# actionml/universal-recommender

Hardware: NVIDIA H100
Metric: CCO train events/sec to indicator model (higher is better)
Workload: dtype int32+f64

## Files before the change

universal_recommender_b200/csrc/cco_api.cu:

```cuda
#include <cuda_runtime.h>
#include <dlfcn.h>
#include <stdarg.h>
#include <stdio.h>
#include <stdlib.h>
#include <string.h>

#include <algorithm>
#include <charconv>
#include <cmath>
#include <functional>
#include <cub/cub.cuh>
#include <nvtx3/nvToolsExt.h>
#include <condition_variable>
#include <mutex>
#include <string>
#include <thread>
#include <unordered_map>
#include <vector>

#include "../../include/cco_b200.h"
#include "cco_kernels.cuh"
#include "cco_sampler.cuh"
#include "cco_format.cuh"
#include "cco_strings.cuh"
#include "cco_json.cuh"
#include "cco_events.cuh"
#include "cco_queries.cuh"
#include "cco_results.cuh"
#include "cco_index_pages.cuh"
#include "cco_index_write.cuh"
#include "cco_refresh.cuh"
#include "cco_intern.cuh"

namespace cco {

static thread_local char g_err[512] = "";
static int set_error(int code, const char *fmt, ...) {
  va_list ap;
  va_start(ap, fmt);
  vsnprintf(g_err, sizeof g_err, fmt, ap);
  va_end(ap);
  return code;
}
#define CK(expr)                                                                                      \
  do {                                                                                                \
    cudaError_t _e = (expr);                                                                          \
    if (_e != cudaSuccess)                                                                            \
      return set_error(_e == cudaErrorMemoryAllocation ? CCO_E_OOM : CCO_E_CUDA, "%s: %s (%s:%d)", #expr, \
                       cudaGetErrorString(_e), __FILE__, __LINE__);                                   \
  } while (0)
#define CKR(expr)            \
  do {                       \
    int _r = (expr);         \
    if (_r != CCO_OK) return _r; \
  } while (0)

typedef struct ncclComm *ncclComm_t;
typedef struct { char internal[128]; } ncclUniqueId;
struct Nccl {
  void *h = nullptr;
  int (*GetUniqueId)(ncclUniqueId *) = nullptr;
  int (*CommInitRank)(ncclComm_t *, int, ncclUniqueId, int) = nullptr;
  int (*CommInitAll)(ncclComm_t *, int, const int *) = nullptr;
  int (*CommDestroy)(ncclComm_t) = nullptr;
  int (*AllReduce)(const void *, void *, size_t, int, int, ncclComm_t, cudaStream_t) = nullptr;
  int (*AllGather)(const void *, void *, size_t, int, ncclComm_t, cudaStream_t) = nullptr;
  int (*Broadcast)(const void *, void *, size_t, int, int, ncclComm_t, cudaStream_t) = nullptr;
  int (*GroupStart)() = nullptr;
  int (*GroupEnd)() = nullptr;
  const char *(*GetErrorString)(int) = nullptr;
};
static Nccl g_nccl;
static std::mutex g_nccl_mu;
static int load_nccl() {
  std::lock_guard<std::mutex> lk(g_nccl_mu);
  if (g_nccl.h) return CCO_OK;
  void *h = dlopen("libnccl.so.2", RTLD_NOW | RTLD_GLOBAL);
  if (!h) h = dlopen("libnccl.so", RTLD_NOW | RTLD_GLOBAL);
  if (!h) return set_error(CCO_E_NCCL, "cannot load libnccl.so.2: %s", dlerror());
#define SYM(field, name)                                                         \
  *(void **)(&g_nccl.field) = dlsym(h, name);                                    \
  if (!g_nccl.field) return set_error(CCO_E_NCCL, "libnccl: missing symbol %s", name);
  SYM(GetUniqueId, "ncclGetUniqueId")
  SYM(CommInitRank, "ncclCommInitRank")
  SYM(CommInitAll, "ncclCommInitAll")
  SYM(CommDestroy, "ncclCommDestroy")
  SYM(AllReduce, "ncclAllReduce")
  SYM(AllGather, "ncclAllGather")
  SYM(Broadcast, "ncclBroadcast")
  SYM(GroupStart, "ncclGroupStart")
  SYM(GroupEnd, "ncclGroupEnd")
  SYM(GetErrorString, "ncclGetErrorString")
#undef SYM
  g_nccl.h = h;
// ... 324 lines not shown
  c->launches++;
  ar.release(tmp);
  ar.release(kb.Alternate());
  ar.release(vb.Alternate());
  *k = kb.Current();
  *v = vb.Current();
  return CCO_OK;
}
static int bits_for(long long n) {
  int b = 1;
  while ((1LL << b) < n) ++b;
  return b;
}

static int keys_to_csr(cco_ctx *c, Arena &ar, unsigned long long *k0, unsigned long long *k1, long long n, int bits, long long n_valid,
                       long long n_rows, int32_t *col, long long *rp, long long *n_unique) {
  cudaStream_t s = c->stream;
  cub::DoubleBuffer<unsigned long long> db(k0, k1);
  size_t tb = 0;
  CK(cub::DeviceRadixSort::SortKeys(nullptr, tb, db, n, 0, bits, s));
  void *tmp;
  CKR(ar.alloc((char **)&tmp, tb));
  CK(cub::DeviceRadixSort::SortKeys(tmp, tb, db, n, 0, bits, s));
  ar.release(tmp);
  unsigned long long *sorted = db.Current(), *other = db.Alternate();
  uint32_t *flag, *pos;
  CKR(ar.alloc(&flag, n_valid + 1));
  CKR(ar.alloc(&pos, n_valid + 1));
  CK(cudaMemsetAsync(flag + n_valid, 0, 4, s));
  k_unique_flags<<<grid_for(n_valid, 256, c->sm_count), 256, 0, s>>>(n_valid, sorted, flag);
  CKR(exclusive_sum(c, ar, flag, pos, n_valid + 1));
  uint32_t nuq = 0;
  CKR(mail_fetch(c, &nuq, pos + n_valid, 4));
  k_unique_scatter<<<grid_for(n_valid, 256, c->sm_count), 256, 0, s>>>(n_valid, sorted, flag, pos, other, col);
  CKR(mail_wait(c));
  k_rowptr_from_keys<<<grid_for(n_rows + 1, 256, c->sm_count), 256, 0, s>>>(n_rows, nuq, other, rp);
  c->launches += 3;
  ar.release(flag);
  ar.release(pos);
  *n_unique = nuq;
  return CCO_OK;
}

static int canonicalize_device(cco_ctx *c, Arena &ar, DevRaw &m) {
  if (m.nnz == 0) return CCO_OK;
  unsigned long long *k0, *k1;
  CKR(ar.alloc(&k0, m.nnz));
  CKR(ar.alloc(&k1, m.nnz));
  k_expand_keys<<<grid_for(m.n_rows * kSG, 256, c->sm_count), 256, 0, c->stream>>>(m.n_rows, m.rp, m.col, k0);
  c->launches++;
  long long n_unique = 0;
  CKR(keys_to_csr(c, ar, k0, k1, m.nnz, 32 + bits_for(m.n_rows), m.nnz, m.n_rows, m.col + m.q_base, m.rp, &n_unique));
  m.col += m.q_base;
  m.q_base = 0;
  m.nnz = n_unique;
  CK(cudaGetLastError());
  ar.release(k0);
  ar.release(k1);
  return CCO_OK;
}

struct HeavyRows {
  int32_t *list = nullptr;
  int *n = nullptr;
};
static int list_heavy_rows(cco_ctx *c, Arena &ar, const DevRaw &raw, HeavyRows *h) {
  CKR(ar.alloc(&h->list, std::max<long long>(raw.n_rows, 1)));
  CKR(ar.alloc(&h->n, 1));
  CK(cudaMemsetAsync(h->n, 0, 4, c->stream));
  if (raw.n_rows > 0) {
    k_list_heavy_rows<<<grid_for(raw.n_rows, 256, c->sm_count), 256, 0, c->stream>>>(raw.n_rows, raw.rp, h->list, h->n);
    c->launches++;
  }
  return CCO_OK;
}
static void launch_check(cco_ctx *c, const DevRaw &raw, const HeavyRows &h, int *flags) {
  if (raw.n_rows <= 0) return;
  const long long q_lo = raw.q_base, q_hi = raw.q_base + raw.nnz;
  k_check_rows<kSG><<<grid_for(raw.n_rows * kSG, 256, c->sm_count), 256, 0, c->stream>>>(raw.n_rows, raw.n_cols, raw.rp, raw.col, q_lo, q_hi,
                                                                                       nullptr, nullptr, flags);
  k_check_rows<32><<<c->sm_count * 4, 256, 0, c->stream>>>(raw.n_rows, raw.n_cols, raw.rp, raw.col, q_lo, q_hi, h.list, h.n, flags);
  c->launches += 2;
}
struct SampleScratch {
  unsigned long long *col_thr = nullptr;
  uint8_t *keep = nullptr;
};
static int sample_scratch(cco_ctx *c, Arena &ar, const DevRaw &raw, const int32_t *raw_counts, int32_t m, SampleScratch *sc) {
  CKR(ar.alloc(&sc->col_thr, std::max<int32_t>(raw.n_cols, 1)));
  CKR(ar.alloc(&sc->keep, std::max<long long>(raw.nnz, 1)));
  if (raw.n_cols > 0) {
    k_col_thresholds<<<grid_for(raw.n_cols, 256, c->sm_count, 4), 256, 0, c->stream>>>(raw.n_cols, raw_counts, m, sc->col_thr);
    c->launches++;
  }
  return CCO_OK;
}
static void launch_count(cco_ctx *c, const DevRaw &raw, const SampleScratch &sc, int32_t m, int32_t seed, uint32_t flags, const int *bad,
                         uint32_t *kept, int32_t *new_counts) {
  if (raw.n_rows <= 0 || raw.nnz <= 0) return;
  const long long q_lo = raw.q_base, q_hi = raw.q_base + raw.nnz;
  const long long n_chunks = (raw.nnz + kSampleChunk - 1) / kSampleChunk;
  k_sample_count<<<grid_for(n_chunks * 32, 256, c->sm_count), 256, 0, c->stream>>>(raw.n_rows, raw.row_base, raw.rp, raw.col, raw.n_cols, q_lo, q_hi,
                                                                                  sc.col_thr, m, seed, flags, bad, kept, new_counts, sc.keep);
  c->launches++;
}
static int launch_write(cco_ctx *c, Arena &ar, const DevRaw &raw, const SampleScratch &sc, int32_t *dst) {
  if (raw.n_rows <= 0 || raw.nnz <= 0) return CCO_OK;
  long long *n_sel;
  CKR(ar.alloc(&n_sel, 1));
  size_t tb = 0;
  CK(cub::DeviceSelect::Flagged(nullptr, tb, raw.col + raw.q_base, sc.keep, dst, n_sel, (long long)raw.nnz, c->stream));
  void *tmp;
  CKR(ar.alloc((char **)&tmp, tb));
  CK(cub::DeviceSelect::Flagged(tmp, tb, raw.col + raw.q_base, sc.keep, dst, n_sel, (long long)raw.nnz, c->stream));
  ar.release(tmp);
  c->launches += 2;
  return CCO_OK;
}

constexpr int kHistCopies = 16;
static bool hist_fits_smem(const cco_ctx *c, int32_t n_cols) { return ((size_t)n_cols + 1) / 2 * 4 <= c->smem_optin; }
static int count_raw_columns(cco_ctx *c, Arena &ar, const std::vector<DevRaw> &raw, const std::vector<long long> &col_off, const cudaEvent_t *ready,
                             int *verdict, int32_t **counts_out) {
  cudaStream_t s = c->stream;
  const int n_mats = (int)raw.size();
  const long long total_cols = col_off[n_mats];
  const long long copy_stride = std::max<long long>(total_cols, 1);
  bool copies = false;
  for (int i = 0; i < n_mats; ++i) copies = copies || (raw[i].n_rows > 0 && !hist_fits_smem(c, raw[i].n_cols));
  const int n_copies = copies ? kHistCopies : 1;
  int32_t *counts;
  CKR(ar.alloc(&counts, (size_t)copy_stride * n_copies));
  CK(cudaMemsetAsync(counts, 0, sizeof(int32_t) * (size_t)copy_stride * n_copies, s));
  *counts_out = counts;
  std::vector<int> fit;
  for (int i = 0; i < n_mats; ++i)
    if (raw[i].n_rows > 0 && hist_fits_smem(c, raw[i].n_cols)) fit.push_back(i);
  for (size_t b0 = 0; b0 < fit.size(); b0 += kHistSegs) {
    const size_t b1 = std::min(fit.size(), b0 + kHistSegs);
    HistBatch hb{};
    long long nnz_sum = 0;
    int32_t max_cols = 0;
    for (size_t t = b0; t < b1; ++t) {
      nnz_sum += raw[fit[t]].nnz;
      max_cols = std::max(max_cols, raw[fit[t]].n_cols);
    }
    const size_t smem = ((size_t)max_cols + 1) / 2 * 4;
    const int per_sm = std::max(1, std::min<int>(2048 / kHistThreads, (int)(c->smem_optin / std::max<size_t>(smem + 1024, 1))));
    const long long target = (long long)c->sm_count * per_sm;
    for (size_t t = b0; t < b1; ++t) {
      const int i = fit[t];
      if (ready) CK(cudaStreamWaitEvent(s, ready[i], 0));
      const long long share = nnz_sum > 0 ? (target * raw[i].nnz + nnz_sum - 1) / nnz_sum : 1;
      const long long need = (raw[i].nnz + kHistMinEntries - 1) / kHistMinEntries;
      HistSeg &g = hb.seg[hb.n++];
      g.col = raw[i].col + raw[i].q_base;
      g.rp = raw[i].rp;
      g.nnz = raw[i].nnz;
      g.n_rows = raw[i].n_rows;
      g.q_lo = raw[i].q_base;
      g.q_hi = raw[i].q_base + raw[i].nnz;
      g.counts = counts + col_off[i];
      g.verdict = verdict ? verdict + 2 * i : nullptr;
      g.n_cols = raw[i].n_cols;
      g.cta0 = hb.cta_end;
      hb.cta_end += (int32_t)std::max(1LL, std::min(share, need));
    }
    CK(cudaFuncSetAttribute(k_col_counts_smem, cudaFuncAttributeMaxDynamicSharedMemorySize, (int)smem));
    k_col_counts_smem<<<hb.cta_end, kHistThreads, smem, s>>>(hb);
    c->launches++;
  }
  for (int i = 0; i < n_mats && copies; ++i) {
    if (raw[i].n_rows == 0 || hist_fits_smem(c, raw[i].n_cols)) continue;
    if (ready) CK(cudaStreamWaitEvent(s, ready[i], 0));
    int *v = verdict ? verdict + 2 * i : nullptr;
    if (v) {
      k_check_row_ptr<<<grid_for(raw[i].n_rows, 256, c->sm_count), 256, 0, s>>>(raw[i].n_rows, raw[i].rp, raw[i].q_base, raw[i].q_base + raw[i].nnz, v);
      c->launches++;
    }
    if (raw[i].nnz > 0) {
      k_col_histogram_flat<true><<<grid_for(raw[i].nnz, 256, c->sm_count), 256, 0, s>>>(raw[i].nnz, raw[i].col + raw[i].q_base, raw[i].n_cols,
                                                                                       counts + col_off[i], kHistCopies, copy_stride, v);
      c->launches++;
    }
  }
  if (copies) {
    k_sum_copies<<<grid_for(total_cols, 256, c->sm_count), 256, 0, s>>>(total_cols, kHistCopies, copy_stride, counts);
    c->launches++;
  }
  if (ready)
    for (int i = 0; i < n_mats; ++i) CK(cudaStreamWaitEvent(s, ready[i], 0));
  return CCO_OK;
}

static int nccl_check(int rc, const char *what) {
  if (rc != 0) return set_error(CCO_E_NCCL, "%s: %s", what, g_nccl.GetErrorString(rc));
  return CCO_OK;
}

static int downsample_all(cco_ctx *c, Arena &ar, const std::vector<DevRaw> &raw, const int *d_check , long long U,
                          const int32_t *raw_counts, int32_t *marg_all, const std::vector<long long> &col_off,
                          const cco_indicator_params_t *params, int32_t seed, uint32_t flags, std::vector<DevMat> &dm,
                          const cudaEvent_t *stage_ev ) {
  cudaStream_t s = c->stream;
  const int W = c->world, r = c->rank, n_mats = (int)raw.size();
  const long long S = (U + W - 1) / W;
  std::vector<uint32_t *> kept(n_mats, nullptr);
  std::vector<SampleScratch> sc(n_mats);
  for (int i = 0; i < n_mats; ++i) {
    DevMat *out = &dm[i];
    out->n_rows = U;
    out->n_cols = raw[i].n_cols;
    out->marg = marg_all + col_off[i];
    CKR(ar.alloc(&kept[i], (size_t)(W * S + 1)));
    CKR(ar.alloc(&out->rp, U + 1));
    CK(cudaMemsetAsync(kept[i], 0, sizeof(uint32_t) * (size_t)(W * S + 1), s));
    CKR(sample_scratch(c, ar, raw[i], raw_counts + col_off[i], params[i].max_interactions, &sc[i]));
    launch_count(c, raw[i], sc[i], params[i].max_interactions, seed, flags, d_check + 2 * i, kept[i], out->marg);
  }
  CK(cudaEventRecord(stage_ev[0], s));
  if (W > 1) {
    if (S > 0) {
      g_nccl.GroupStart();
      for (int i = 0; i < n_mats; ++i) {
        int rc = g_nccl.AllGather(kept[i] + (size_t)r * S, kept[i], (size_t)S, kNcclUint32, c->comm, s);
        if (rc != 0) { g_nccl.GroupEnd(); return nccl_check(rc, "ncclAllGather(kept counts)"); }
      }
      CKR(nccl_check(g_nccl.GroupEnd(), "ncclGroupEnd(kept counts)"));
    }
    if (col_off[n_mats] > 0)
      CKR(nccl_check(g_nccl.AllReduce(marg_all, marg_all, (size_t)col_off[n_mats], kNcclInt32, kNcclSum, c->comm, s), "ncclAllReduce(marginals)"));
  }
  std::vector<uint32_t> edge((size_t)n_mats * (W + 1), 0);
  for (int i = 0; i < n_mats; ++i) {
    CKR(exclusive_sum(c, ar, kept[i], dm[i].rp, U + 1));
    ar.release(kept[i]);
    if (W > 1)
      for (int q = 0; q <= W; ++q) CKR(mail_fetch(c, &edge[(size_t)i * (W + 1) + q], dm[i].rp + std::min<long long>((long long)q * S, U), 4));
  }
  CK(cudaEventRecord(stage_ev[1], s));
  if (W > 1) CKR(mail_wait(c));
  std::vector<long long> cap(n_mats, 0);
  std::vector<int32_t *> gathered(n_mats, nullptr);
  for (int i = 0; i < n_mats; ++i) {
    if (W == 1) {
      CKR(ar.alloc(&dm[i].col, std::max<long long>(raw[i].nnz, 1)));
      CKR(launch_write(c, ar, raw[i], sc[i], dm[i].col));
    } else {
      for (int q = 0; q < W; ++q) cap[i] = std::max<long long>(cap[i], (long long)edge[(size_t)i * (W + 1) + q + 1] - edge[(size_t)i * (W + 1) + q]);
      CKR(ar.alloc(&dm[i].col, std::max<long long>(edge[(size_t)i * (W + 1) + W], 1)));
      if (cap[i] > 0) {
        CKR(ar.alloc(&gathered[i], (size_t)(cap[i] * W)));
        CKR(launch_write(c, ar, raw[i], sc[i], gathered[i] + (size_t)r * cap[i]));
      }
    }
    ar.release(sc[i].col_thr);
    ar.release(sc[i].keep);
  }
  CK(cudaEventRecord(stage_ev[2], s));
  if (W > 1) {
    g_nccl.GroupStart();
    for (int i = 0; i < n_mats; ++i) {
      if (!gathered[i]) continue;
      int rc = g_nccl.AllGather(gathered[i] + (size_t)r * cap[i], gathered[i], (size_t)cap[i], kNcclInt32, c->comm, s);
      if (rc != 0) { g_nccl.GroupEnd(); return nccl_check(rc, "ncclAllGather(column blocks)"); }
    }
    CKR(nccl_check(g_nccl.GroupEnd(), "ncclGroupEnd(column blocks)"));
    for (int i = 0; i < n_mats; ++i) {
      if (!gathered[i]) continue;
      dim3 grid((unsigned)std::max(1, std::min(c->sm_count * 8 / W, 1024)), (unsigned)W);
      k_pack_blocks<<<grid, 256, 0, s>>>(W, S, U, cap[i], dm[i].rp, gathered[i], dm[i].col);
      c->launches++;
      ar.release(gathered[i]);
    }
  }
  CK(cudaEventRecord(stage_ev[3], s));
  CK(cudaGetLastError());
  return CCO_OK;
}


struct BinCfg {
  int group;
  int slots;
  int cap;
  int cbuf;
  int caux, keep_max, final_max;
  bool dense;
  bool bitmap;
  bool sorted;
  int bm_words;
  size_t region;
  size_t smem;
  int ctas_per_sm;
};

static int next_pow2(int x) {
  int p = 1;
  while (p < x) p <<= 1;
  return p;
}

template <int GROUP>
static int launch_rows_t(cco_ctx *c, const RowArgs &a, BinCfg &cfg, cudaStream_t st) {
  constexpr int CTA = GROUP == 32 ? 64 : GROUP;
  int occ = 1;
  void (*kern)(const RowArgs) = cfg.dense ? k_rows<GROUP, true> : k_rows<GROUP, false>;
  if constexpr (GROUP == 512 || GROUP == 256)
    if (cfg.bitmap) kern = k_rows<GROUP, false, true>;
  if constexpr (GROUP == 32)
    if (cfg.sorted) kern = k_rows<32, false, false, true>;
  CK(cudaFuncSetAttribute(kern, cudaFuncAttributeMaxDynamicSharedMemorySize, (int)cfg.smem));
  CK(cudaOccupancyMaxActiveBlocksPerMultiprocessor(&occ, kern, CTA, cfg.smem));
  kern<<<c->sm_count * std::max(occ, 1) * 4, CTA, cfg.smem, st>>>(a);
  cfg.ctas_per_sm = occ;
  c->launches++;
  CK(cudaGetLastError());
  return CCO_OK;
}
static int launch_rows(cco_ctx *c, const RowArgs &a, BinCfg &cfg, cudaStream_t st) {
  switch (cfg.group) {
    case 1024: return launch_rows_t<1024>(c, a, cfg, st);
    case 512: return launch_rows_t<512>(c, a, cfg, st);
    case 256: return launch_rows_t<256>(c, a, cfg, st);
    case 128: return launch_rows_t<128>(c, a, cfg, st);
    case 32: return launch_rows_t<32>(c, a, cfg, st);
  }
  return set_error(CCO_E_INVALID_ARG, "internal: bad bin config");
}

static BinCfg make_cfg(cco_ctx *c, int group, int want_slots, int top_k, int n_cols_b) {
  BinCfg f;
  const int groups = group == 32 ? 2 : 1;
  f.group = group;
  f.final_max = next_pow2(top_k);
  f.cbuf = next_pow2(top_k + std::max(group, 128) + (group == 32 ? 64 : 0));
  if (group == 32 && top_k + 32 <= 96) f.cbuf = 128;
  f.keep_max = std::max(f.final_max, (f.cbuf - group) / 2);
  f.caux = group == 32 ? 0 : f.keep_max;
  size_t fixed = (size_t)(f.cbuf + f.caux) * 16 + 2 * 256 + 512 + 1024 + (size_t)(group / 32) * 256;
  size_t avail = (c->smem_optin - 1024) / groups;
// ... 6038 lines not shown
    if (len[i] < 1 || len[i] > 32) return set_error(CCO_E_CUDA, "text %lld has length %d", (long long)i, len[i]);
    memcpy(bytes + offsets[i], slot.data() + 32 * (size_t)i, (size_t)len[i]);
    offsets[i + 1] = offsets[i] + len[i];
  }
  return CCO_OK;
}

int cco_debug_downsample(cco_ctx_t *c, const cco_csr_t *m, int32_t max_interactions, int32_t seed, uint32_t flags,
                         int64_t **row_ptr, int32_t **col_idx, int32_t *raw_col_counts, int32_t *new_col_counts) {
  if (!c || !m || !row_ptr || !col_idx) return set_error(CCO_E_INVALID_ARG, "null argument");
  if (c->world != 1 || !c->members.empty()) return set_error(CCO_E_UNSUPPORTED, "debug entries need a single-GPU context");
  cco_indicator_params_t prm = {max_interactions, 1, 0, 0.0};
  CKR(validate_host(1, m, &prm));
  CK(cudaSetDevice(c->device));
  mail_reset(c);
  c->ev_timing_used = c->ev_plain_used = 0;
  cco_dataset *ds = nullptr;
  CKR(dataset_upload(c, 1, m, flags, &ds));
  struct DG { cco_dataset *d; ~DG() { dataset_release(d); } } dg{ds};
  Arena ar(c->stream);
  Prepared p;
  CKR(prepare(c, ar, ds, &prm, seed, flags, &p));
  const DevMat &dm = p.dm[0];
  std::vector<uint32_t> rp32((size_t)m->n_rows + 1);
  CK(cudaMemcpyAsync(rp32.data(), dm.rp, sizeof(uint32_t) * rp32.size(), cudaMemcpyDeviceToHost, c->stream));
  if (raw_col_counts && m->n_cols > 0)
    CK(cudaMemcpyAsync(raw_col_counts, p.raw_counts, sizeof(int32_t) * (size_t)m->n_cols, cudaMemcpyDeviceToHost, c->stream));
  if (new_col_counts && m->n_cols > 0)
    CK(cudaMemcpyAsync(new_col_counts, dm.marg, sizeof(int32_t) * (size_t)m->n_cols, cudaMemcpyDeviceToHost, c->stream));
  CK(cudaStreamSynchronize(c->stream));
  CK(cudaGetLastError());
  size_t nnz = rp32[m->n_rows];
  int64_t *rp = (int64_t *)malloc(sizeof(int64_t) * rp32.size());
  int32_t *ci = (int32_t *)calloc(std::max<size_t>(nnz, 1), sizeof(int32_t));
  if (!rp || !ci) return set_error(CCO_E_OOM, "malloc failed");
  for (size_t i = 0; i < rp32.size(); ++i) rp[i] = rp32[i];
  const size_t n_copy = std::min<size_t>(nnz, (size_t)ds->nnz[0]);
  if (n_copy) CK(cudaMemcpy(ci, dm.col, sizeof(int32_t) * n_copy, cudaMemcpyDeviceToHost));
  *row_ptr = rp;
  *col_idx = ci;
  return CCO_OK;
}

int cco_debug_downsample_block(cco_ctx_t *c, const cco_csr_t *m, int64_t row_lo, int64_t row_hi, const int32_t *raw_col_counts,
                               int32_t max_interactions, int32_t seed, uint32_t flags, int64_t *kept_per_row, int32_t **col_idx,
                               int32_t *new_col_counts) {
  if (!c || !m || !col_idx || (m->n_rows > 0 && !kept_per_row) || (m->n_cols > 0 && (!raw_col_counts || !new_col_counts)))
    return set_error(CCO_E_INVALID_ARG, "null argument");
  if (c->world != 1 || !c->members.empty()) return set_error(CCO_E_UNSUPPORTED, "debug entries need a single-GPU context");
  cco_indicator_params_t prm = {max_interactions, 1, 0, 0.0};
  CKR(validate_host(1, m, &prm));
  if (row_lo < 0 || row_hi < row_lo || row_hi > m->n_rows)
    return set_error(CCO_E_INVALID_ARG, "rows [%lld, %lld) outside [0, %lld)", (long long)row_lo, (long long)row_hi, (long long)m->n_rows);
  CK(cudaSetDevice(c->device));
  mail_reset(c);
  cudaStream_t s = c->stream;
  cco_dataset *ds = nullptr;
  CKR(dataset_upload(c, 1, m, flags, &ds));
  struct DG { cco_dataset *d; ~DG() { dataset_release(d); } } dg{ds};
  Arena ar(s);
  const long long U = ds->n_users;
  const int32_t width = std::max<int32_t>(m->n_cols, 1);
  long long q[2] = {0, 0};
  CK(cudaMemcpyAsync(&q[0], ds->rp[0] + row_lo, sizeof(long long), cudaMemcpyDeviceToHost, s));
  CK(cudaMemcpyAsync(&q[1], ds->rp[0] + row_hi, sizeof(long long), cudaMemcpyDeviceToHost, s));
  CK(cudaStreamSynchronize(s));
  DevRaw blk;
  blk.n_rows = row_hi - row_lo;
  blk.row_base = row_lo;
  blk.n_cols = m->n_cols;
  blk.q_base = q[0];
  blk.nnz = q[1] - q[0];
  blk.rp = ds->rp[0] + row_lo;
  blk.col = ds->col[0];
  int32_t *counts, *marg, *dst;
  uint32_t *kept;
  CKR(ar.alloc(&counts, width));
  CKR(ar.alloc(&marg, width));
  CKR(ar.alloc(&kept, U + 1));
  CKR(ar.alloc(&dst, std::max<long long>(blk.nnz, 1)));
  if (m->n_cols > 0) CK(cudaMemcpyAsync(counts, raw_col_counts, sizeof(int32_t) * (size_t)m->n_cols, cudaMemcpyHostToDevice, s));
  CK(cudaMemsetAsync(marg, 0, sizeof(int32_t) * (size_t)width, s));
  CK(cudaMemsetAsync(kept, 0, sizeof(uint32_t) * ((size_t)U + 1), s));
  SampleScratch sc;
  CKR(sample_scratch(c, ar, blk, counts, max_interactions, &sc));
  launch_count(c, blk, sc, max_interactions, seed, flags, nullptr, kept, marg);
  CKR(launch_write(c, ar, blk, sc, dst));
  std::vector<uint32_t> hk((size_t)U + 1);
  CK(cudaMemcpyAsync(hk.data(), kept, sizeof(uint32_t) * hk.size(), cudaMemcpyDeviceToHost, s));
  if (m->n_cols > 0) CK(cudaMemcpyAsync(new_col_counts, marg, sizeof(int32_t) * (size_t)m->n_cols, cudaMemcpyDeviceToHost, s));
  CK(cudaStreamSynchronize(s));
  CK(cudaGetLastError());
  size_t n_kept = 0;
  for (long long r = 0; r < U; ++r) {
    kept_per_row[r] = hk[r];
    if (r >= row_lo && r < row_hi) n_kept += hk[r];
  }
  int32_t *ci = (int32_t *)calloc(std::max<size_t>(n_kept, 1), sizeof(int32_t));
  if (!ci) return set_error(CCO_E_OOM, "malloc failed");
  const size_t n_copy = std::min<size_t>(n_kept, (size_t)blk.nnz);
  if (n_copy) {
    cudaError_t e = cudaMemcpy(ci, dst, sizeof(int32_t) * n_copy, cudaMemcpyDeviceToHost);
    if (e != cudaSuccess) {
      free(ci);
      return set_error(CCO_E_CUDA, "cudaMemcpy: %s", cudaGetErrorString(e));
    }
  }
  *col_idx = ci;
  return CCO_OK;
}

int cco_debug_key_range_cap(cco_ctx_t *c, int32_t max_keys) {
  if (!c || max_keys < 0) return set_error(CCO_E_INVALID_ARG, "null context or negative cap");
  c->key_range_cap = max_keys;
  for (cco_ctx *m : c->members) m->key_range_cap = max_keys;
  return CCO_OK;
}

int cco_debug_intern_hash_bits(cco_ctx_t *c, int32_t bits) {
  if (!c || bits < 0 || bits > 64) return set_error(CCO_E_INVALID_ARG, "null context or hash bits %d not in [0, 64]", bits);
  c->intern_mask = bits == 64 ? ~0ULL : (1ULL << bits) - 1;
  return CCO_OK;
}

int cco_debug_cooccurrence(cco_ctx_t *c, const cco_csr_t *a, const cco_csr_t *b, int64_t **row_ptr, int32_t **col_idx,
                           int32_t **count) {
  if (!c || !a || !b || !row_ptr || !col_idx || !count) return set_error(CCO_E_INVALID_ARG, "null argument");
  if (c->world != 1 || !c->members.empty()) return set_error(CCO_E_UNSUPPORTED, "debug entries need a single-GPU context");
  cco_csr_t two[2] = {*a, *b};
  cco_indicator_params_t prm[2] = {{0x7fffffff, 1, 0, 0.0}, {0x7fffffff, 1, 0, 0.0}};
  CKR(validate_host(2, two, prm));
  CK(cudaSetDevice(c->device));
  mail_reset(c);
  c->ev_timing_used = c->ev_plain_used = 0;
  cco_dataset *ds = nullptr;
  CKR(dataset_upload(c, 2, two, 0, &ds));
  struct DG { cco_dataset *d; ~DG() { dataset_release(d); } } dg{ds};
  Arena ar(c->stream);
  struct CopyJoin {
    cco_ctx *c;
    ~CopyJoin() { cudaStreamSynchronize(c->copy_stream); }
  } copy_join{c};
  Prepared prep;
  CKR(prepare(c, ar, ds, prm, 0, 0, &prep));
  const int32_t n_items_a = prep.dm[0].n_cols;
  ResultMat rm;
  IndicatorOut io;
  IndicatorState ist;
  struct EG { IndicatorState &x; ~EG() { if (x.packed) cudaEventDestroy(x.packed); } } eg{ist};
  cco_indicator_params_t p1 = {0x7fffffff, 1, 0, 0.0};
  auto put = [&]() {
    for (void *p : {(void *)rm.row_ptr, (void *)rm.col, (void *)rm.llr, (void *)rm.cnt})
      if (p) c->pinned_put(p);
  };
  int rc = enqueue_indicator(c, ar, prep.at_ptr, prep.at_users, n_items_a, prep.dm[0].marg, prep.max_marg[0], prep.max_marg[1], prep.dm[1],
                             a->n_rows, false, p1, 0, true, nullptr, nullptr, nullptr, &ist);
  if (rc == CCO_OK) rc = finish_indicator(c, &ist, 0, 0, &rm, &io);
  cudaStreamSynchronize(c->copy_stream);
  if (rc != CCO_OK) {
    put();
    return rc;
  }
  size_t nnz = (size_t)rm.row_ptr[n_items_a];
  int64_t *rp = (int64_t *)malloc(sizeof(int64_t) * ((size_t)n_items_a + 1));
  int32_t *ci = (int32_t *)malloc(sizeof(int32_t) * std::max<size_t>(nnz, 1));
  int32_t *cn = (int32_t *)malloc(sizeof(int32_t) * std::max<size_t>(nnz, 1));
  if (!rp || !ci || !cn) {
    put();
    return set_error(CCO_E_OOM, "malloc failed");
  }
// ... 1376 lines not shown
```

universal_recommender_b200/csrc/cco_sampler.cuh:

```cuda
#pragma once

#include <cuda_runtime.h>
#include <stdint.h>

#include "cco_kernels.cuh"

namespace cco {

constexpr int kSampleChunk = 256;

template <typename P>
__device__ __forceinline__ long long warp_find_row(const P *__restrict__ rp, long long n_rows, long long q, int lane) {
  long long lo = 0, hi = n_rows;
  while (hi - lo > 1) {
    const long long step = (hi - lo + 31) / 32;
    const long long p = lo + lane * step;
    const bool ok = p < hi && (long long)rp[p] <= q;
    const unsigned b = __ballot_sync(0xffffffffu, ok) | 1u;
    const int top = 31 - __clz(b);
    lo += top * step;
    hi = hi < lo + step ? hi : lo + step;
  }
  return lo;
}

__global__ void __launch_bounds__(256) k_sample_count(long long n_rows, long long row_base, const long long *__restrict__ rp,
                                                      const int32_t *__restrict__ col, int32_t n_cols, long long q_lo, long long q_hi,
                                                      const unsigned long long *__restrict__ col_thr, int32_t m, int32_t seed, uint32_t flags,
                                                      const int *__restrict__ bad ,
                                                      uint32_t *__restrict__ kept_per_row , int32_t *__restrict__ new_counts,
                                                      uint8_t *__restrict__ keep_flag) {
  const int lane = threadIdx.x & 31;
  const long long warp = (blockIdx.x * (long long)blockDim.x + threadIdx.x) >> 5;
  const long long n_warps = ((long long)gridDim.x * blockDim.x) >> 5;
  const long long n_chunks = (q_hi - q_lo + kSampleChunk - 1) / kSampleChunk;
  const bool intdiv = (flags & CCO_FLAG_ROWRATE_INTDIV) != 0;
  const long long kNoRow = 0x7fffffffffffffffLL;
  if (n_rows <= 0) return;
  if (bad && *bad) {
    for (long long q = blockIdx.x * (long long)blockDim.x + threadIdx.x; q < q_hi - q_lo; q += (long long)gridDim.x * blockDim.x) keep_flag[q] = 0;
    return;
  }
  for (long long chunk = warp; chunk < n_chunks; chunk += n_warps) {
    const long long Q0 = q_lo + chunk * kSampleChunk;
    const long long Q1 = Q0 + kSampleChunk < q_hi ? Q0 + kSampleChunk : q_hi;
    long long base = warp_find_row(rp, n_rows, Q0, lane);
    long long start_i, end_i;
    unsigned long long t_i, x_i;
    uint32_t kept_i;
#define CCO_LOAD_WINDOW()                                                                                   \
  {                                                                                                         \
    const long long r = base + lane;                                                                        \
    start_i = end_i = kNoRow;                                                                               \
    t_i = kKeepAlways;                                                                                      \
    x_i = 0;                                                                                                \
    if (r < n_rows) {                                                                                       \
      start_i = rp[r];                                                                                      \
      end_i = rp[r + 1];                                                                                    \
      const long long d = end_i - start_i;                                                                  \
      if (d > (long long)m) t_i = rate_threshold(row_sample_rate(d, m, intdiv));  \
      x_i = mix64(((uint64_t)(uint32_t)seed << 32) | (uint64_t)(uint32_t)(row_base + r));                   \
    }                                                                                                       \
    kept_i = 0;                                                                                             \
  }
#define CCO_FLUSH_WINDOW()                                                                                  \
  if (kept_i) atomicAdd(&kept_per_row[row_base + base + lane], kept_i);
    CCO_LOAD_WINDOW()
    for (long long qb = Q0; qb < Q1; qb += 32) {
      const long long q = qb + lane;
      bool pending = q < Q1;
      const int32_t j = pending ? col[q] : 0;
      unsigned long long t_col = kKeepAlways;
      if (pending && (uint32_t)j < (uint32_t)n_cols) t_col = col_thr[j];
      while (true) {
        int idx = 0;
#pragma unroll
        for (int step = 16; step > 0; step >>= 1) {
          const long long v = __shfl_sync(0xffffffffu, end_i, idx + step - 1);
          if (v <= q) idx += step;
        }
        {
          const long long v = __shfl_sync(0xffffffffu, end_i, idx);
          if (v <= q) idx += 1;
        }
        const int src = idx & 31;
        const unsigned long long t_row = __shfl_sync(0xffffffffu, t_i, src);
        const unsigned long long x_row = __shfl_sync(0xffffffffu, x_i, src);
        const bool here = pending && idx < 32;
        const bool real_row = base + idx < n_rows;
        bool keep = false;
        if (here) {
          keep = real_row && (uint32_t)j < (uint32_t)n_cols && keep_entry_thr(t_row, t_col, x_row, (uint32_t)j);
          keep_flag[q - q_lo] = keep ? 1 : 0;
          if (keep && new_counts) atomicAdd(&new_counts[j], 1);
        }
        const unsigned kb = __ballot_sync(0xffffffffu, keep);
        const int a = start_i <= qb ? 0 : (start_i >= qb + 32 ? 32 : (int)(start_i - qb));
        const int b = end_i <= qb ? 0 : (end_i >= qb + 32 ? 32 : (int)(end_i - qb));
        if (b > a) {
          const unsigned below_b = b >= 32 ? 0xffffffffu : ((1u << b) - 1u);
          const unsigned below_a = (1u << a) - 1u;
          kept_i += __popc(kb & below_b & ~below_a);
        }
        pending = pending && !here;
        if (!__any_sync(0xffffffffu, pending)) break;
        CCO_FLUSH_WINDOW()
        base += 32;
        if (base >= n_rows) {
          if (pending) keep_flag[q - q_lo] = 0;
          kept_i = 0;
          start_i = end_i = kNoRow;
          break;
        }
        CCO_LOAD_WINDOW()
      }
      if (base >= n_rows) {
        for (long long q2 = qb + 32 + lane; q2 < Q1; q2 += 32) keep_flag[q2 - q_lo] = 0;
        break;
      }
    }
    if (base < n_rows && base + lane < n_rows) { CCO_FLUSH_WINDOW() }
#undef CCO_LOAD_WINDOW
#undef CCO_FLUSH_WINDOW
  }
}

__global__ void k_check_row_ptr(long long n_rows, const long long *__restrict__ rp, long long q_lo, long long q_hi, int *flags) {
  int bad = 0;
  for (long long r = blockIdx.x * (long long)blockDim.x + threadIdx.x; r < n_rows; r += (long long)gridDim.x * blockDim.x) {
    const long long s = rp[r], e = rp[r + 1];
    if (e < s || s < q_lo || e > q_hi) bad = 1;
  }
  if (bad) atomicOr(&flags[0], 1);
}
template <bool AGG>
__global__ void k_col_histogram_flat(long long n, const int32_t *__restrict__ col, int32_t n_cols, int32_t *__restrict__ counts, int n_copies,
                                     long long copy_stride, int *flags ) {
  int32_t *mine = counts + (long long)(blockIdx.x % n_copies) * copy_stride;
  const int lane = threadIdx.x & 31;
  int bad = 0;
  for (long long q0 = blockIdx.x * (long long)blockDim.x + (threadIdx.x & ~31); q0 < n; q0 += (long long)gridDim.x * blockDim.x) {
    const long long q = q0 + lane;
    const bool act = q < n;
    const int32_t j = act ? col[q] : -1;
    const bool ok = act && (uint32_t)j < (uint32_t)n_cols;
    if (act && !ok) bad = 1;
    if (AGG) {
      const unsigned om = __ballot_sync(0xffffffffu, ok);
      if (ok) {
        const unsigned peers = __match_any_sync(om, j);
        if ((__ffs(peers) - 1) == lane) atomicAdd(&mine[j], __popc(peers));
      }
    } else if (ok) {
      atomicAdd(&mine[j], 1);
    }
  }
  if (flags && bad) atomicOr(&flags[0], 1);
}

__global__ void __launch_bounds__(256) k_transpose_entries(long long n_rows, const uint32_t *__restrict__ rp, const int32_t *__restrict__ col,
                                                           uint32_t *__restrict__ cursor, int32_t *__restrict__ users) {
  if (n_rows <= 0) return;
  const int lane = threadIdx.x & 31;
  const long long warp = (blockIdx.x * (long long)blockDim.x + threadIdx.x) >> 5;
  const long long n_warps = ((long long)gridDim.x * blockDim.x) >> 5;
  const long long nnz = rp[n_rows];
  const long long n_chunks = (nnz + kSampleChunk - 1) / kSampleChunk;
  for (long long chunk = warp; chunk < n_chunks; chunk += n_warps) {
    const long long Q0 = chunk * kSampleChunk;
    const long long Q1 = Q0 + kSampleChunk < nnz ? Q0 + kSampleChunk : nnz;
    long long base = warp_find_row(rp, n_rows, Q0, lane);
    long long end_i = base + lane < n_rows ? (long long)rp[base + lane + 1] : 0x7fffffffffffffffLL;
    for (long long qb = Q0; qb < Q1; qb += 32) {
      const long long q = qb + lane;
      bool pending = q < Q1;
      const int32_t j = pending ? col[q] : 0;
      while (true) {
        int idx = 0;
#pragma unroll
        for (int step = 16; step > 0; step >>= 1) {
          const long long v = __shfl_sync(0xffffffffu, end_i, idx + step - 1);
          if (v <= q) idx += step;
        }
        if (__shfl_sync(0xffffffffu, end_i, idx & 31) <= q) idx += 1;
        const bool here = pending && idx < 32;
        if (here) users[atomicAdd(&cursor[j], 1u)] = (int32_t)(base + idx);
        pending = pending && !here;
        if (!__any_sync(0xffffffffu, pending)) break;
        base += 32;
        end_i = base + lane < n_rows ? (long long)rp[base + lane + 1] : 0x7fffffffffffffffLL;
      }
    }
  }
}

constexpr int kHistSegs = 8;
constexpr int kHistThreads = 1024;
constexpr long long kHistMinEntries = 1 << 16;
struct HistSeg {
  const int32_t *col;
  const long long *rp;
  long long nnz, n_rows, q_lo, q_hi;
  int32_t *counts;
  int *verdict;
  int32_t n_cols;
  int32_t cta0;
// ... 52 lines not shown
```

Measured before the change: 4.409 billion.

## Batch downsampling across matrices with bitmask keep flags and custom compaction kernel

Replaces the per-matrix threshold, count and cub select-flagged launches with batched kernels that handle up to eight matrices per launch. Keep flags become per-chunk 32-bit bitmasks with per-chunk counts, and a new write kernel compacts kept columns using an exclusive sum of those counts. Row-pointer scans for all matrices are merged into a single segmented scan-by-key, and column loads are software-prefetched two iterations ahead in the count kernel. This aims to cut launch count and byte-per-entry flag traffic, at the cost of more complex chunk-to-segment mapping and contiguous per-warp chunk ranges.

```diff
diff --git a/universal_recommender_b200/csrc/cco_api.cu b/universal_recommender_b200/csrc/cco_api.cu
--- a/universal_recommender_b200/csrc/cco_api.cu
+++ b/universal_recommender_b200/csrc/cco_api.cu
@@ -10,6 +10,8 @@
 #include <cmath>
 #include <functional>
 #include <cub/cub.cuh>
+#include <thrust/iterator/counting_iterator.h>
+#include <thrust/iterator/transform_iterator.h>
 #include <nvtx3/nvToolsExt.h>
 #include <condition_variable>
 #include <mutex>
@@ -500,39 +502,71 @@
   k_check_rows<32><<<c->sm_count * 4, 256, 0, c->stream>>>(raw.n_rows, raw.n_cols, raw.rp, raw.col, q_lo, q_hi, h.list, h.n, flags);
   c->launches += 2;
 }
-struct SampleScratch {
-  unsigned long long *col_thr = nullptr;
-  uint8_t *keep = nullptr;
+struct SamplePlan {
+  std::vector<SampleBatch> batches;
+  std::vector<int> mat;
+  long long n_chunks = 0;
+  unsigned long long *thr = nullptr;
+  uint32_t *bits = nullptr, *cnt = nullptr, *off = nullptr;
 };
-static int sample_scratch(cco_ctx *c, Arena &ar, const DevRaw &raw, const int32_t *raw_counts, int32_t m, SampleScratch *sc) {
-  CKR(ar.alloc(&sc->col_thr, std::max<int32_t>(raw.n_cols, 1)));
-  CKR(ar.alloc(&sc->keep, std::max<long long>(raw.nnz, 1)));
-  if (raw.n_cols > 0) {
-    k_col_thresholds<<<grid_for(raw.n_cols, 256, c->sm_count, 4), 256, 0, c->stream>>>(raw.n_cols, raw_counts, m, sc->col_thr);
-    c->launches++;
-  }
-  return CCO_OK;
-}
-static void launch_count(cco_ctx *c, const DevRaw &raw, const SampleScratch &sc, int32_t m, int32_t seed, uint32_t flags, const int *bad,
-                         uint32_t *kept, int32_t *new_counts) {
-  if (raw.n_rows <= 0 || raw.nnz <= 0) return;
-  const long long q_lo = raw.q_base, q_hi = raw.q_base + raw.nnz;
-  const long long n_chunks = (raw.nnz + kSampleChunk - 1) / kSampleChunk;
-  k_sample_count<<<grid_for(n_chunks * 32, 256, c->sm_count), 256, 0, c->stream>>>(raw.n_rows, raw.row_base, raw.rp, raw.col, raw.n_cols, q_lo, q_hi,
-                                                                                  sc.col_thr, m, seed, flags, bad, kept, new_counts, sc.keep);
-  c->launches++;
-}
-static int launch_write(cco_ctx *c, Arena &ar, const DevRaw &raw, const SampleScratch &sc, int32_t *dst) {
-  if (raw.n_rows <= 0 || raw.nnz <= 0) return CCO_OK;
-  long long *n_sel;
-  CKR(ar.alloc(&n_sel, 1));
-  size_t tb = 0;
-  CK(cub::DeviceSelect::Flagged(nullptr, tb, raw.col + raw.q_base, sc.keep, dst, n_sel, (long long)raw.nnz, c->stream));
-  void *tmp;
-  CKR(ar.alloc((char **)&tmp, tb));
-  CK(cub::DeviceSelect::Flagged(tmp, tb, raw.col + raw.q_base, sc.keep, dst, n_sel, (long long)raw.nnz, c->stream));
-  ar.release(tmp);
-  c->launches += 2;
+static int sample_count(cco_ctx *c, Arena &ar, const std::vector<DevRaw> &raw, const std::vector<long long> &col_off, const int32_t *raw_counts,
+                        const cco_indicator_params_t *params, int32_t seed, uint32_t flags, const int *bad, uint32_t *kept, long long kept_stride,
+                        int32_t *new_counts, SamplePlan *p) {
+  cudaStream_t s = c->stream;
+  for (int i = 0; i < (int)raw.size(); ++i) {
+    if (raw[i].n_rows <= 0 || raw[i].nnz <= 0) continue;
+    if (p->batches.empty() || p->batches.back().n == kSampleSegs) p->batches.emplace_back();
+    SampleBatch &b = p->batches.back();
+    SampleSeg &g = b.seg[b.n++];
+    p->mat.push_back(i);
+    g.rp = raw[i].rp;
+    g.col = raw[i].col;
+    g.bad = bad ? bad + 2 * i : nullptr;
+    g.kept = kept + i * kept_stride;
+    g.new_counts = new_counts + col_off[i];
+    g.n_rows = raw[i].n_rows;
+    g.row_base = raw[i].row_base;
+    g.q_lo = raw[i].q_base;
+    g.q_hi = raw[i].q_base + raw[i].nnz;
+    g.chunk0 = p->n_chunks;
+    g.col0 = col_off[i];
+    g.n_cols = raw[i].n_cols;
+    g.m = params[i].max_interactions;
+    p->n_chunks += (raw[i].nnz + kSampleChunk - 1) / kSampleChunk;
+    b.chunk_end = p->n_chunks;
+  }
+  CKR(ar.alloc(&p->thr, std::max<long long>(col_off.back(), 1)));
+  CKR(ar.alloc(&p->bits, std::max<long long>(p->n_chunks * (kSampleChunk / 32), 1)));
+  CKR(ar.alloc(&p->cnt, std::max<long long>(p->n_chunks, 1)));
+  for (const SampleBatch &b : p->batches) {
+    int32_t max_cols = 0;
+    for (int t = 0; t < b.n; ++t) max_cols = std::max(max_cols, b.seg[t].n_cols);
+    if (max_cols > 0) {
+      k_sample_thresholds<<<dim3(grid_for(max_cols, 256, c->sm_count, 4), b.n), 256, 0, s>>>(b, raw_counts, p->thr);
+      c->launches++;
+    }
+    k_sample_count<<<grid_for((b.chunk_end - b.seg[0].chunk0) * 32, 256, c->sm_count, 3), 256, 0, s>>>(b, p->thr, seed, flags, p->bits, p->cnt);
+    c->launches++;
+  }
+  return CCO_OK;
+}
+struct MatOfSlot {
+  long long L;
+  __host__ __device__ int operator()(long long k) const { return (int)(k / L); }
+};
+static int sample_offsets(cco_ctx *c, Arena &ar, SamplePlan *p) {
+  CKR(ar.alloc(&p->off, std::max<long long>(p->n_chunks, 1)));
+  if (p->n_chunks > 0) CKR(exclusive_sum(c, ar, p->cnt, p->off, p->n_chunks));
+  return CCO_OK;
+}
+static int sample_write(cco_ctx *c, Arena &ar, SamplePlan *p, const std::vector<int32_t *> &dst) {
+  size_t t = 0;
+  for (SampleBatch &b : p->batches) {
+    for (int k = 0; k < b.n; ++k) b.seg[k].dst = dst[p->mat[t++]];
+    k_sample_write<<<grid_for((b.chunk_end - b.seg[0].chunk0) * 32, 256, c->sm_count), 256, 0, c->stream>>>(b, p->bits, p->off);
+    c->launches++;
+  }
+  for (void *q : {(void *)p->thr, (void *)p->bits, (void *)p->cnt, (void *)p->off}) ar.release(q);
   return CCO_OK;
 }
 
@@ -623,25 +657,26 @@
   cudaStream_t s = c->stream;
   const int W = c->world, r = c->rank, n_mats = (int)raw.size();
   const long long S = (U + W - 1) / W;
-  std::vector<uint32_t *> kept(n_mats, nullptr);
-  std::vector<SampleScratch> sc(n_mats);
+  const long long L = W * S + 1;
+  uint32_t *kept, *rp_all;
+  CKR(ar.alloc(&kept, (size_t)(n_mats * L)));
+  CKR(ar.alloc(&rp_all, (size_t)(n_mats * L)));
+  CK(cudaMemsetAsync(kept, 0, sizeof(uint32_t) * (size_t)(n_mats * L), s));
   for (int i = 0; i < n_mats; ++i) {
     DevMat *out = &dm[i];
     out->n_rows = U;
     out->n_cols = raw[i].n_cols;
     out->marg = marg_all + col_off[i];
-    CKR(ar.alloc(&kept[i], (size_t)(W * S + 1)));
-    CKR(ar.alloc(&out->rp, U + 1));
-    CK(cudaMemsetAsync(kept[i], 0, sizeof(uint32_t) * (size_t)(W * S + 1), s));
-    CKR(sample_scratch(c, ar, raw[i], raw_counts + col_off[i], params[i].max_interactions, &sc[i]));
-    launch_count(c, raw[i], sc[i], params[i].max_interactions, seed, flags, d_check + 2 * i, kept[i], out->marg);
-  }
+    out->rp = rp_all + i * L;
+  }
+  SamplePlan sp;
+  CKR(sample_count(c, ar, raw, col_off, raw_counts, params, seed, flags, d_check, kept, L, marg_all, &sp));
   CK(cudaEventRecord(stage_ev[0], s));
   if (W > 1) {
     if (S > 0) {
       g_nccl.GroupStart();
       for (int i = 0; i < n_mats; ++i) {
-        int rc = g_nccl.AllGather(kept[i] + (size_t)r * S, kept[i], (size_t)S, kNcclUint32, c->comm, s);
+        int rc = g_nccl.AllGather(kept + i * L + (size_t)r * S, kept + i * L, (size_t)S, kNcclUint32, c->comm, s);
         if (rc != 0) { g_nccl.GroupEnd(); return nccl_check(rc, "ncclAllGather(kept counts)"); }
       }
       CKR(nccl_check(g_nccl.GroupEnd(), "ncclGroupEnd(kept counts)"));
@@ -649,32 +684,39 @@
     if (col_off[n_mats] > 0)
       CKR(nccl_check(g_nccl.AllReduce(marg_all, marg_all, (size_t)col_off[n_mats], kNcclInt32, kNcclSum, c->comm, s), "ncclAllReduce(marginals)"));
   }
+  {
+    auto key = thrust::make_transform_iterator(thrust::counting_iterator<long long>(0), MatOfSlot{L});
+    size_t tb = 0;
+    CK(cub::DeviceScan::ExclusiveSumByKey(nullptr, tb, key, kept, rp_all, n_mats * L, cuda::std::equal_to<>(), s));
+    void *tmp;
+    CKR(ar.alloc((char **)&tmp, tb));
+    CK(cub::DeviceScan::ExclusiveSumByKey(tmp, tb, key, kept, rp_all, n_mats * L, cuda::std::equal_to<>(), s));
+    ar.release(tmp);
+    ar.release(kept);
+  }
+  CKR(sample_offsets(c, ar, &sp));
   std::vector<uint32_t> edge((size_t)n_mats * (W + 1), 0);
-  for (int i = 0; i < n_mats; ++i) {
-    CKR(exclusive_sum(c, ar, kept[i], dm[i].rp, U + 1));
-    ar.release(kept[i]);
-    if (W > 1)
+  if (W > 1)
+    for (int i = 0; i < n_mats; ++i)
       for (int q = 0; q <= W; ++q) CKR(mail_fetch(c, &edge[(size_t)i * (W + 1) + q], dm[i].rp + std::min<long long>((long long)q * S, U), 4));
-  }
   CK(cudaEventRecord(stage_ev[1], s));
   if (W > 1) CKR(mail_wait(c));
   std::vector<long long> cap(n_mats, 0);
-  std::vector<int32_t *> gathered(n_mats, nullptr);
+  std::vector<int32_t *> gathered(n_mats, nullptr), dst(n_mats, nullptr);
   for (int i = 0; i < n_mats; ++i) {
     if (W == 1) {
       CKR(ar.alloc(&dm[i].col, std::max<long long>(raw[i].nnz, 1)));
-      CKR(launch_write(c, ar, raw[i], sc[i], dm[i].col));
+      dst[i] = dm[i].col;
     } else {
       for (int q = 0; q < W; ++q) cap[i] = std::max<long long>(cap[i], (long long)edge[(size_t)i * (W + 1) + q + 1] - edge[(size_t)i * (W + 1) + q]);
       CKR(ar.alloc(&dm[i].col, std::max<long long>(edge[(size_t)i * (W + 1) + W], 1)));
       if (cap[i] > 0) {
         CKR(ar.alloc(&gathered[i], (size_t)(cap[i] * W)));
-        CKR(launch_write(c, ar, raw[i], sc[i], gathered[i] + (size_t)r * cap[i]));
+        dst[i] = gathered[i] + (size_t)r * cap[i];
       }
     }
-    ar.release(sc[i].col_thr);
-    ar.release(sc[i].keep);
-  }
+  }
+  CKR(sample_write(c, ar, &sp, dst));
   CK(cudaEventRecord(stage_ev[2], s));
   if (W > 1) {
     g_nccl.GroupStart();
@@ -6879,10 +6921,10 @@
   if (m->n_cols > 0) CK(cudaMemcpyAsync(counts, raw_col_counts, sizeof(int32_t) * (size_t)m->n_cols, cudaMemcpyHostToDevice, s));
   CK(cudaMemsetAsync(marg, 0, sizeof(int32_t) * (size_t)width, s));
   CK(cudaMemsetAsync(kept, 0, sizeof(uint32_t) * ((size_t)U + 1), s));
-  SampleScratch sc;
-  CKR(sample_scratch(c, ar, blk, counts, max_interactions, &sc));
-  launch_count(c, blk, sc, max_interactions, seed, flags, nullptr, kept, marg);
-  CKR(launch_write(c, ar, blk, sc, dst));
+  SamplePlan sp;
+  CKR(sample_count(c, ar, {blk}, {0, (long long)m->n_cols}, counts, &prm, seed, flags, nullptr, kept, U + 1, marg, &sp));
+  CKR(sample_offsets(c, ar, &sp));
+  CKR(sample_write(c, ar, &sp, {dst}));
   std::vector<uint32_t> hk((size_t)U + 1);
   CK(cudaMemcpyAsync(hk.data(), kept, sizeof(uint32_t) * hk.size(), cudaMemcpyDeviceToHost, s));
   if (m->n_cols > 0) CK(cudaMemcpyAsync(new_col_counts, marg, sizeof(int32_t) * (size_t)m->n_cols, cudaMemcpyDeviceToHost, s));
diff --git a/universal_recommender_b200/csrc/cco_sampler.cuh b/universal_recommender_b200/csrc/cco_sampler.cuh
--- a/universal_recommender_b200/csrc/cco_sampler.cuh
+++ b/universal_recommender_b200/csrc/cco_sampler.cuh
@@ -24,27 +24,73 @@
   return lo;
 }
 
-__global__ void __launch_bounds__(256) k_sample_count(long long n_rows, long long row_base, const long long *__restrict__ rp,
-                                                      const int32_t *__restrict__ col, int32_t n_cols, long long q_lo, long long q_hi,
-                                                      const unsigned long long *__restrict__ col_thr, int32_t m, int32_t seed, uint32_t flags,
-                                                      const int *__restrict__ bad ,
-                                                      uint32_t *__restrict__ kept_per_row , int32_t *__restrict__ new_counts,
-                                                      uint8_t *__restrict__ keep_flag) {
+constexpr int kSampleSegs = 8;
+struct SampleSeg {
+  const long long *rp;
+  const int32_t *col;
+  const int *bad;
+  uint32_t *kept;
+  int32_t *new_counts;
+  int32_t *dst;
+  long long n_rows, row_base, q_lo, q_hi;
+  long long chunk0;
+  long long col0;
+  int32_t n_cols, m;
+};
+struct SampleBatch {
+  SampleSeg seg[kSampleSegs];
+  int32_t n;
+  long long chunk_end;
+};
+__device__ __forceinline__ int sample_seg_of(const SampleBatch &b, long long chunk) {
+  int i = 0;
+  while (i + 1 < b.n && chunk >= b.seg[i + 1].chunk0) ++i;
+  return i;
+}
+
+__global__ void k_sample_thresholds(const __grid_constant__ SampleBatch b, const int32_t *__restrict__ raw_counts,
+                                    unsigned long long *__restrict__ thr) {
+  const SampleSeg &s = b.seg[blockIdx.y];
+  for (int j = blockIdx.x * blockDim.x + threadIdx.x; j < s.n_cols; j += gridDim.x * blockDim.x) {
+    const int32_t c = raw_counts[s.col0 + j];
+    thr[s.col0 + j] = c <= s.m ? kKeepAlways : rate_threshold(__ddiv_rn((double)s.m, (double)c));
+  }
+}
+
+__global__ void __launch_bounds__(256, 3) k_sample_count(const __grid_constant__ SampleBatch b, const unsigned long long *__restrict__ thr,
+                                                         int32_t seed, uint32_t flags, uint32_t *__restrict__ keep_bits,
+                                                         uint32_t *__restrict__ chunk_kept) {
+  constexpr int kWords = kSampleChunk / 32;
   const int lane = threadIdx.x & 31;
   const long long warp = (blockIdx.x * (long long)blockDim.x + threadIdx.x) >> 5;
   const long long n_warps = ((long long)gridDim.x * blockDim.x) >> 5;
-  const long long n_chunks = (q_hi - q_lo + kSampleChunk - 1) / kSampleChunk;
   const bool intdiv = (flags & CCO_FLAG_ROWRATE_INTDIV) != 0;
   const long long kNoRow = 0x7fffffffffffffffLL;
-  if (n_rows <= 0) return;
-  if (bad && *bad) {
-    for (long long q = blockIdx.x * (long long)blockDim.x + threadIdx.x; q < q_hi - q_lo; q += (long long)gridDim.x * blockDim.x) keep_flag[q] = 0;
-    return;
-  }
-  for (long long chunk = warp; chunk < n_chunks; chunk += n_warps) {
-    const long long Q0 = q_lo + chunk * kSampleChunk;
-    const long long Q1 = Q0 + kSampleChunk < q_hi ? Q0 + kSampleChunk : q_hi;
-    long long base = warp_find_row(rp, n_rows, Q0, lane);
+  const long long c0 = b.seg[0].chunk0, per_warp = (b.chunk_end - c0 + n_warps - 1) / n_warps;
+  const long long g_end = c0 + (warp + 1) * per_warp < b.chunk_end ? c0 + (warp + 1) * per_warp : b.chunk_end;
+  for (long long g = c0 + warp * per_warp; g < g_end;) {
+    const int si = sample_seg_of(b, g);
+    const SampleSeg &s = b.seg[si];
+    const long long seg_end = si + 1 < b.n ? b.seg[si + 1].chunk0 : b.chunk_end;
+    const long long g1 = seg_end < g_end ? seg_end : g_end;
+    if (s.bad && *s.bad) {
+      for (; g < g1; ++g) {
+        if (lane < kWords) keep_bits[g * kWords + lane] = 0;
+        if (lane == 0) chunk_kept[g] = 0;
+      }
+      continue;
+    }
+    const long long n_rows = s.n_rows, row_base = s.row_base;
+    const long long *__restrict__ rp = s.rp;
+    const int32_t *__restrict__ col = s.col;
+    const unsigned long long *__restrict__ col_thr = thr + s.col0;
+    const int32_t n_cols = s.n_cols, m = s.m;
+    uint32_t *__restrict__ kept_per_row = s.kept;
+    int32_t *__restrict__ new_counts = s.new_counts;
+    long long Qc = s.q_lo + (g - s.chunk0) * kSampleChunk;
+    const long long Q1 = s.q_lo + (g1 - s.chunk0) * kSampleChunk < s.q_hi ? s.q_lo + (g1 - s.chunk0) * kSampleChunk : s.q_hi;
+    uint32_t word = 0, n_kept = 0;
+    long long base = warp_find_row(rp, n_rows, Qc, lane);
     long long start_i, end_i;
     unsigned long long t_i, x_i;
     uint32_t kept_i;
@@ -66,12 +112,18 @@
 #define CCO_FLUSH_WINDOW()                                                                                  \
   if (kept_i) atomicAdd(&kept_per_row[row_base + base + lane], kept_i);
     CCO_LOAD_WINDOW()
-    for (long long qb = Q0; qb < Q1; qb += 32) {
+    int32_t j_next = Qc + lane < Q1 ? col[Qc + lane] : 0;
+    int32_t j_after = Qc + 32 + lane < Q1 ? col[Qc + 32 + lane] : 0;
+    unsigned long long t_next = Qc + lane < Q1 && (uint32_t)j_next < (uint32_t)n_cols ? col_thr[j_next] : kKeepAlways;
+    for (long long qb = Qc; qb < Q1; qb += 32) {
       const long long q = qb + lane;
       bool pending = q < Q1;
-      const int32_t j = pending ? col[q] : 0;
-      unsigned long long t_col = kKeepAlways;
-      if (pending && (uint32_t)j < (uint32_t)n_cols) t_col = col_thr[j];
+      const int32_t j = j_next;
+      const unsigned long long t_col = t_next;
+      j_next = j_after;
+      t_next = q + 32 < Q1 && (uint32_t)j_next < (uint32_t)n_cols ? col_thr[j_next] : kKeepAlways;
+      j_after = q + 64 < Q1 ? col[q + 64] : 0;
+      uint32_t kw = 0;
       while (true) {
         int idx = 0;
 #pragma unroll
@@ -91,14 +143,14 @@
         bool keep = false;
         if (here) {
           keep = real_row && (uint32_t)j < (uint32_t)n_cols && keep_entry_thr(t_row, t_col, x_row, (uint32_t)j);
-          keep_flag[q - q_lo] = keep ? 1 : 0;
           if (keep && new_counts) atomicAdd(&new_counts[j], 1);
         }
         const unsigned kb = __ballot_sync(0xffffffffu, keep);
+        kw |= kb;
         const int a = start_i <= qb ? 0 : (start_i >= qb + 32 ? 32 : (int)(start_i - qb));
-        const int b = end_i <= qb ? 0 : (end_i >= qb + 32 ? 32 : (int)(end_i - qb));
-        if (b > a) {
-          const unsigned below_b = b >= 32 ? 0xffffffffu : ((1u << b) - 1u);
+        const int bb = end_i <= qb ? 0 : (end_i >= qb + 32 ? 32 : (int)(end_i - qb));
+        if (bb > a) {
+          const unsigned below_b = bb >= 32 ? 0xffffffffu : ((1u << bb) - 1u);
           const unsigned below_a = (1u << a) - 1u;
           kept_i += __popc(kb & below_b & ~below_a);
         }
@@ -107,21 +159,58 @@
         CCO_FLUSH_WINDOW()
         base += 32;
         if (base >= n_rows) {
-          if (pending) keep_flag[q - q_lo] = 0;
           kept_i = 0;
           start_i = end_i = kNoRow;
           break;
         }
         CCO_LOAD_WINDOW()
       }
-      if (base >= n_rows) {
-        for (long long q2 = qb + 32 + lane; q2 < Q1; q2 += 32) keep_flag[q2 - q_lo] = 0;
-        break;
-      }
+      if (lane == (int)((qb - Qc) >> 5)) word = kw;
+      n_kept += __popc(kw);
+      const bool tail = base >= n_rows;
+      if (tail || qb + 32 >= Qc + kSampleChunk || qb + 32 >= Q1) {
+        if (lane < kWords) keep_bits[g * kWords + lane] = word;
+        if (lane == 0) chunk_kept[g] = n_kept;
+        ++g;
+        Qc += kSampleChunk;
+        word = n_kept = 0;
+      }
+      if (tail) break;
     }
     if (base < n_rows && base + lane < n_rows) { CCO_FLUSH_WINDOW() }
 #undef CCO_LOAD_WINDOW
 #undef CCO_FLUSH_WINDOW
+    for (; g < g1; ++g) {
+      if (lane < kWords) keep_bits[g * kWords + lane] = 0;
+      if (lane == 0) chunk_kept[g] = 0;
+    }
+  }
+}
+
+__global__ void __launch_bounds__(256) k_sample_write(const __grid_constant__ SampleBatch b, const uint32_t *__restrict__ keep_bits,
+                                                      const uint32_t *__restrict__ chunk_off) {
+  constexpr int kWords = kSampleChunk / 32;
+  const int lane = threadIdx.x & 31;
+  const long long warp = (blockIdx.x * (long long)blockDim.x + threadIdx.x) >> 5;
+  const long long n_warps = ((long long)gridDim.x * blockDim.x) >> 5;
+  const unsigned below = (1u << lane) - 1u;
+  for (long long g = b.seg[0].chunk0 + warp; g < b.chunk_end; g += n_warps) {
+    const SampleSeg &s = b.seg[sample_seg_of(b, g)];
+    const int32_t *__restrict__ src = s.col + s.q_lo + (g - s.chunk0) * kSampleChunk + lane;
+    const uint32_t mine = lane < kWords ? keep_bits[g * kWords + lane] : 0u;
+    uint32_t w[kWords];
+    int32_t v[kWords];
+#pragma unroll
+    for (int k = 0; k < kWords; ++k) {
+      w[k] = __shfl_sync(0xffffffffu, mine, k);
+      if ((w[k] >> lane) & 1u) v[k] = src[32 * k];
+    }
+    uint32_t o = chunk_off[g] - chunk_off[s.chunk0];
+#pragma unroll
+    for (int k = 0; k < kWords; ++k) {
+      if ((w[k] >> lane) & 1u) s.dst[o + __popc(w[k] & below)] = v[k];
+      o += __popc(w[k]);
+    }
   }
 }
 
```

After: 4.493 billion (median of 6 runs). About the same (+1.9%).
